# kfkq/DQMC

Measured on AMD Instinct MI355X. Metric: MC sweeps/sec, 2D Hubbard N=256 Ltau=200, higher is better.
Workload: dtype f64; 1 GPU; cfg3: 16x16 Hubbard U=8.0 beta=8.0 Ltau=200 n_stab=10 t=1 mu=-0.1; chains_per_gpu=1, n_chains_total=1, parallelism=independent chains, 1 gpu x 1 chain

## Files before the change

### dqmc_amd/csrc/common.h

```cpp
#pragma once

#include <hip/hip_runtime.h>
#include <cstdint>
#include <memory>
#include <string>

struct dqmc_engine;

namespace dq {

constexpr int WAVE = 64;

void set_error(const std::string& msg);
const char* get_error();

#define DQ_HIP(call)                                                                    \
    do {                                                                                \
        hipError_t _e = (call);                                                         \
        if (_e != hipSuccess) {                                                         \
            ::dq::set_error(std::string(#call) + ": " + hipGetErrorString(_e));         \
            return -2;                                              \
        }                                                                               \
    } while (0)

// ... 22 lines not shown
    double* p = nullptr;
    long stride = 0;
    __host__ __device__ double* at(int c) const { return p + (long)c * stride; }
};
struct CMat {
    const double* p = nullptr;
    long stride = 0;
    CMat() = default;
    __host__ __device__ CMat(const double* p_, long s) : p(p_), stride(s) {}
    __host__ __device__ CMat(const Mat& m) : p(m.p), stride(m.stride) {}
    __host__ __device__ const double* at(int c) const { return p + (long)c * stride; }
};
using Vec = Mat;
using CVec = CMat;

struct GemmDesc {
    CMat A, B;
    Mat C;
    Mat CT{nullptr, 0};
    CVec rs, ks, cs;
    int n = 0;
    int transA = 0;
    int accumulate = 0;
};
int launch_gemm(const GemmDesc& g, int n_chains, hipStream_t s);

int launch_build_expv(const int8_t* fields, long f_stride, int nt, int n, const double* tab_expv ,
                      double* expv, double* invexpv, long v_stride, int n_chains, hipStream_t s);
int launch_split_d(CVec d, Vec dl_inv, Vec ds, double* logsum, int n, int n_chains, hipStream_t s);
int launch_split_d2(CVec d1, Vec dl1, Vec ds1, CVec d2, Vec dl2, Vec ds2, int n, int n_chains, hipStream_t s);
int launch_measure_equal_time(CMat G, double* out, long out_stride, int L1, int L2, int accumulate, int n_chains, hipStream_t s);
int launch_measure_unequal_time(const double* Gtt, const double* Gt0, const double* G0t, double* out, long out_stride, int L1, int L2, int nt,
                                int accumulate, int n_chains, hipStream_t s);
int launch_axpb_identity(CMat in, Mat out, double a, double b, int n, int n_chains, hipStream_t s);
int launch_copy(CMat in, Mat out, long count, int n_chains, hipStream_t s);
int launch_set_identity(Mat out, int n, int n_chains, hipStream_t s);
int launch_transpose_scale(CMat in, Mat out, CVec rs, int n, int n_chains, hipStream_t s);
int launch_max_abs_diff(CMat A, CMat B, double* err, long err_stride, int n, int n_chains, hipStream_t s);
int launch_add_scaled_cols(CMat A, CMat B, CVec cs, Mat C, int n, int n_chains, hipStream_t s);
int launch_scale_rows(CMat in, CVec rs, Mat out, int n, int n_chains, hipStream_t s);
struct DevStats { double acc_rate, max_err, sum_err, n_err; long long n_accepted, n_proposed; };
int launch_fold_stats(DevStats* st, const int* acc, long acc_stride, int n_slices, const double* err, long err_stride, int n_err,
                      int n, int nt, int n_chains, hipStream_t s);

struct QrWork {
    double* tau; long tau_stride;
// ... 11 lines not shown
int launch_qr_panel(Mat A, Mat L, QrWork w, int n, int n_chains, hipStream_t s);
long qrcp_coop_sync_granules(int n);
int qrcp_coop_workgroups(int n, int n_chains);
enum class QrFamily { Panel, ColumnOwner, Cooperative, Streaming };
int launch_to_ldr(QrFamily f, Mat A, Mat L, Vec d, Mat R, QrWork w, int n, int n_chains, hipStream_t s);

int launch_lu_blocked(Mat A, int* perm, long perm_stride, int* rowpos, long rowpos_stride, double* logabsdet, int accumulate_logdet,
                      int* info, int n, int n_chains, hipStream_t s);
int launch_lu_solve(CMat LU, const int* perm, long perm_stride, Mat X, CVec dg, int mode, int n, int n_chains, hipStream_t s);

int launch_tri_solve(CMat R, const int* perm, long perm_stride, Mat X, CVec dg, double* scratch, long scratch_stride, int n, int n_chains, hipStream_t s);

bool gj_fused_fits(int n);
bool gj_fused_default(int n);
int launch_gj_solve(Mat A, Mat B, Mat X, Mat SA, double* tinv, int* perm, long perm_stride, int* rowpos, int* rowpos_alt, long rowpos_stride,
                    double* logabsdet, int accumulate_logdet, int* info, int n, int n_chains, bool fused, hipStream_t s);

struct UpdateTables {
    double rb[4][3];
    double delta[4][3];
    double ev[4];
    double iev[4];
    double pad[32];
};
struct UpdateDesc {
    Mat G;
    int8_t* fields; long f_stride;
    double* expv; double* invexpv; long v_stride;
    const UpdateTables* tabs;
    const int32_t* perm; const uint8_t* kprop; const double* u; long rs_stride;
    double* Upanel; double* Wpanel; long panel_stride;
    double* Cpanel = nullptr;
    int* state; long state_stride;
    double* prep; long prep_stride;
    Mat GT{nullptr, 0};
    int gt_valid = 0;
    void* slice_sync = nullptr;
    unsigned slice_epoch = 0;
    int slice_absent_tile = -1;
    int slice_absent_l = -1;
    int slice_late_tile = -1, slice_late_us = 0;
    int* info = nullptr;
    int* acc_out; long acc_stride;
    int n, nt;
};
constexpr int UPDATE_KD = 32;

struct SliceSync {
    unsigned long long seq; unsigned int error; unsigned int solo_count; unsigned int pad[12];
    unsigned int arrive[496];
};
constexpr size_t SLICE_SYNC_BYTES = 2048;
static_assert(sizeof(SliceSync) == SLICE_SYNC_BYTES, "SliceSync layout");
constexpr unsigned SLICE_EPOCH_LIMIT = 1u << 24;
constexpr unsigned SLICE_SOLO_BIT = 1u << 30, SLICE_FINAL_BIT = 1u << 31;
__host__ __device__ inline unsigned slice_tag(unsigned epoch, unsigned window) { return (epoch << 8) | window; }
enum class SlicePath { PersistentWalk, PersistentSubmatrix, Solo, Pairs, PairsTailSolo };
int launch_update_slice(SlicePath path, const UpdateDesc& d, int l, int acc_slot, int n_chains, hipStream_t s);
int launch_update_slice_sm(const UpdateDesc& d, int l, int acc_slot, int n_chains, hipStream_t s);
int slice_flush_workgroups(int n);
bool slice_reserve(int device, int n, int n_chains);
void slice_release(int device, int n, int n_chains);
int launch_rank1(Mat G, int i, double delta, double* scratch , long scratch_stride, int n, int n_chains, hipStream_t s);

int launch_rng_fill(int32_t* perm, uint8_t* kprop, double* u, int n, int nt, unsigned long long seed, unsigned first_chain, unsigned h,
                    int n_chains, hipStream_t s);

// ... 24 lines not shown
```

### dqmc_amd/csrc/engine.hip

```cpp
#include "common.h"
#include "../../include/dqmc_hip.h"

#include <cmath>
#include <cstdlib>
#include <cstring>
#include <map>
#include <memory>
#include <mutex>
#include <vector>

namespace dq {

static thread_local std::string g_err;
void set_error(const std::string& msg) { g_err = msg; }
const char* get_error() { return g_err.c_str(); }

int init_device_kernels(int device) {
    static std::mutex mu; static bool done[64] = {};
    std::lock_guard<std::mutex> lk(mu);
    if (device < 0 || device >= 64) { set_error("device ordinal out of range"); return -1; }
    if (done[device]) return 0;
    DQ_HIP(hipSetDevice(device));
    DQ_TRY(update_init_device()); DQ_TRY(update_sm_init_device()); DQ_TRY(qr_init_device()); DQ_TRY(qr_colown_init_device());
    done[device] = true;
    return 0;
}

struct Switches { bool qr_panel; int qr_panel_fused, gj_fused; bool qr_streaming, walk_submatrix, lu_classic, slice_multikernel; };
static const Switches& switches() {
    static const Switches sw = [] {
        const char* panel = getenv("DQMC_QR_PANEL");
        const char* fused = getenv("DQMC_QR_PANEL_FUSED");
        const char* gj = getenv("DQMC_GJ_FUSED");
        return Switches{!(panel && atoi(panel) == 0), fused ? (atoi(fused) != 0 ? 1 : 0) : -1, gj ? (atoi(gj) != 0 ? 1 : 0) : -1, getenv("DQMC_QR_STREAMING") != nullptr, getenv("DQMC_WALK_SUBMATRIX") != nullptr,
                        getenv("DQMC_LU_CLASSIC") != nullptr, getenv("DQMC_SLICE_MULTIKERNEL") != nullptr};
    }();
    return sw;
}

constexpr int GJ_MAX_N = 1024, GJ_MAX_CHAINS = 8;
constexpr int TRI_MAX_N = 640;

static QrFamily pick_qr(int n, int chains, bool allow_panel) {
    const Switches& sw = switches();
    if (sw.qr_streaming) return QrFamily::Streaming;
    if (allow_panel && sw.qr_panel && n >= 64 && n <= 1024 && n % 16 == 0 && chains <= 8) return QrFamily::Panel;
    if (n <= 256) return QrFamily::ColumnOwner;
    return qrcp_coop_workgroups(n, chains) <= 200 ? QrFamily::Cooperative : QrFamily::Streaming;
}

struct KernelPlan {
    QrFamily qr;
    enum class Solve { GaussJordan, BlockedLu } solve;
    enum class Rinv { Blocked, PerColumn } rinv;
    static KernelPlan pick(int n, int chains) {
        return KernelPlan{pick_qr(n, chains, true),
                          n <= GJ_MAX_N && chains <= GJ_MAX_CHAINS && !switches().lu_classic ? Solve::GaussJordan : Solve::BlockedLu,
                          n <= TRI_MAX_N ? Rinv::Blocked : Rinv::PerColumn};
// ... 424 lines not shown
        DQ_TRY(launch_to_ldr(pick_qr(n, S, false), cur, all.L, all.d, all.R, w, n, S, s));
        const LdrRef last = stack.at(S - 1), own = ib.f.at(S - 1);
        DQ_TRY(launch_copy(own.L, last.L, nn, 1, s));
        DQ_TRY(launch_copy(own.R, last.R, nn, 1, s));
        DQ_HIP(hipMemcpyAsync(last.d.p, own.d.p, sizeof(double) * n, hipMemcpyDeviceToDevice, s));
        DQ_HIP(hipMemcpyAsync(last.jpvt, own.jpvt, sizeof(int) * n, hipMemcpyDeviceToDevice, s));
        *last.tri = true; last.touch();
        for (int i = S - 2; i >= 0; --i) DQ_TRY(ctx.ldr_mul_ldr(stack.at(i + 1), ib.f.at(i), stack.at(i)));
        stack_valid = true;
        gt_valid = false;
        return ctx.inv_I_plus_ldr(stack.at(0), mG(), logdet.get());
    }
    int wrap_forward(int l) {
        if (cb) {
            DQ_TRY(cb_apply(mG(), Mat{nullptr, 0}, ctx.T(0), false, false, CVec(), CVec(), CVec(), CVec(), C, 4));
            gt_valid = use_gt();
            return cb_apply(ctx.T(0), Mat{GT.get(), nn}, mG(), false, true, CVec(), CVec(), iev(l), ev(l), C, 4);
        }
        DQ_TRY(ctx.gemm(CMat(expK.get(), nn), mG(), ctx.T(0)));
        gt_valid = use_gt();
        return ctx.gemm(ctx.T(0), CMat(invexpK.get(), nn), mG(), ev(l), CVec(), iev(l), 0, 0, use_gt() ? Mat{GT.get(), nn} : Mat{nullptr, 0});
    }
    bool piggyback() const { return C == 1 && !cb && n <= 256 && pg_eye != nullptr; }
    int wrap_forward_piggy(int l, const double* Pprev, double* Pnext) {
        GemmDesc g; g.A = CMat(expK.get(), 0); g.B = CMat(G.get(), (long)(Pprev - G.get())); g.C = Mat{ctx.T(0).p, (long)(Pnext - ctx.T(0).p)};
        g.rs = CVec(pg_ones.get(), (long)((expv.get() + (long)(l - 1) * n) - pg_ones.get())); g.n = n;
        DQ_TRY(launch_gemm(g, 2, s));
        gt_valid = use_gt();
        return ctx.gemm(ctx.T(0), CMat(invexpK.get(), nn), mG(), ev(l), CVec(), iev(l), 0, 0, use_gt() ? Mat{GT.get(), nn} : Mat{nullptr, 0});
    }
    int wrap_backward_piggy(int l, const double* Pprev, double* Pnext) {
        DQ_TRY(ctx.gemm(CMat(invexpK.get(), nn), mG(), ctx.T(0), CVec(), iev(l)));
        gt_valid = use_gt();
        GemmDesc g; g.A = CMat(ctx.T(0).p, (long)(Pprev - ctx.T(0).p)); g.B = CMat(expK.get(), 0); g.C = Mat{G.get(), (long)(Pnext - G.get())};
        g.ks = CVec(expv.get() + (long)l * n, 0); g.n = n;
        if (use_gt()) g.CT = Mat{GT.get(), (long)(ctx.T(1).p - GT.get())};
        return launch_gemm(g, 2, s);
    }
    int wrap_backward(int l) {
        if (cb) {
            DQ_TRY(cb_apply(mG(), Mat{nullptr, 0}, ctx.T(0), true, true, iev(l), ev(l), CVec(), CVec(), C, 4));
            gt_valid = use_gt();
            return cb_apply(ctx.T(0), Mat{GT.get(), nn}, mG(), true, false, CVec(), CVec(), CVec(), CVec(), C, 4);
        }
        DQ_TRY(ctx.gemm(CMat(invexpK.get(), nn), mG(), ctx.T(0), CVec(), iev(l)));
        gt_valid = use_gt();
        return ctx.gemm(ctx.T(0), CMat(expK.get(), nn), mG(), CVec(), ev(l), CVec(), 0, 0, use_gt() ? Mat{GT.get(), nn} : Mat{nullptr, 0});
    }
    bool use_gt() const { return n <= 256 || slice_path == SlicePath::PersistentSubmatrix; }
    UpdateDesc udesc() const {
        UpdateDesc d; d.G = mG(); d.fields = fields.get(); d.f_stride = (long)nt * n; d.expv = expv.get(); d.invexpv = invexpv.get(); d.v_stride = (long)nt * n;
        d.tabs = tabs.get(); d.perm = rs_perm.get(); d.kprop = rs_k.get(); d.u = rs_u.get(); d.rs_stride = (long)nt * n; d.Upanel = Upanel.get(); d.Wpanel = Wpanel.get(); d.Cpanel = Cpanel.get();
        d.panel_stride = (long)UPDATE_KD * n; d.state = state.get(); d.state_stride = 4; d.prep = prep.get(); d.prep_stride = 4L * n; d.slice_sync = is_persistent(slice_path) ? slice_sync.get() : nullptr; d.slice_epoch = slice_epoch; d.slice_absent_tile = slice_absent_tile; d.slice_absent_l = slice_absent_l; d.slice_late_tile = slice_late_tile; d.slice_late_us = slice_late_us; d.GT = Mat{GT.get(), nn}; d.gt_valid = gt_valid ? 1 : 0; d.info = ctx.info(); d.acc_out = acc.get(); d.acc_stride = nt; d.n = n; d.nt = nt;
        return d;
    }
    int local_update(int l) {
        hipEvent_t e0 = nullptr, e1 = nullptr;
        if (profiling) {
            if (ev_used == ev_pairs.size()) { hipEvent_t a, b; DQ_HIP(hipEventCreate(&a)); DQ_HIP(hipEventCreate(&b)); ev_pairs.emplace_back(a, b); }
            e0 = ev_pairs[ev_used].first; e1 = ev_pairs[ev_used].second; ++ev_used;
            DQ_HIP(hipEventRecord(e0, s));
        }
        if (is_persistent(slice_path)) {
            if (++slice_epoch >= SLICE_EPOCH_LIMIT) { DQ_HIP(hipMemsetAsync(slice_sync.get(), 0, (size_t)C * SLICE_SYNC_BYTES, s)); slice_epoch = 1; }
        }
        DQ_TRY(launch_update_slice(slice_path, udesc(), l, l, C, s));
        if (profiling) DQ_HIP(hipEventRecord(e1, s));
        return 0;
    }
    int check_stream(const char* who, const int32_t* perm, const uint8_t* kprop, const double* u, size_t rows) {
        if (!perm || !kprop || !u) { set_error(std::string(who) + ": null random-stream pointer"); return DQMC_EINVAL; }
        seen.assign((size_t)n, 0);
        for (size_t row = 0; row < rows; ++row) {
            const int32_t* pr = perm + row * n; const uint8_t* kr = kprop + row * n; const unsigned char mark = (unsigned char)(1 + (row & 1));
            if ((row & 1) == 0) std::fill(seen.begin(), seen.end(), 0);
            for (int idx = 0; idx < n; ++idx) {
                const int32_t i = pr[idx];
                if (i < 0 || i >= n || seen[i] == mark || kr[idx] > 2) { set_error(std::string(who) + ": perm is not a permutation of the sites, or kprop > 2"); return DQMC_EINVAL; }
                seen[i] = mark;
            }
        }
        return 0;
    }
    int upload_stream(const int32_t* perm, const uint8_t* kprop, const double* u) {
        const size_t cnt = (size_t)C * nt * n;
        DQ_TRY(check_stream("sweep", perm, kprop, u, (size_t)C * nt));
        DQ_HIP(hipEventSynchronize(stage_free));
        char* base = h_stage.get();
        double* hu = reinterpret_cast<double*>(base);
// ... 1 lines not shown
        uint8_t* hk = reinterpret_cast<uint8_t*>(base + cnt * (sizeof(double) + sizeof(int32_t)));
        std::memcpy(hu, u, cnt * sizeof(double)); std::memcpy(hp, perm, cnt * sizeof(int32_t)); std::memcpy(hk, kprop, cnt);
        DQ_HIP(hipMemcpyAsync(rs_u.get(), hu, cnt * sizeof(double), hipMemcpyHostToDevice, s));
        DQ_HIP(hipMemcpyAsync(rs_perm.get(), hp, cnt * sizeof(int32_t), hipMemcpyHostToDevice, s));
        DQ_HIP(hipMemcpyAsync(rs_k.get(), hk, cnt, hipMemcpyHostToDevice, s));
        DQ_HIP(hipEventRecord(stage_free, s));
        return 0;
    }
    int fill_stream(uint32_t h) {
        return launch_rng_fill(rs_perm.get(), rs_k.get(), rs_u.get(), n, nt, rng_seed, rng_first_chain, h, C, s);
    }
    int stage_stream(const char* who, const int32_t* perm, const uint8_t* kprop, const double* u) {
        if (perm && kprop && u) return upload_stream(perm, kprop, u);
        if (perm || kprop || u) { set_error(std::string(who) + ": pass all three random-stream arrays or none"); return DQMC_EINVAL; }
        if (!rng_seeded) { set_error(std::string(who) + ": null random-stream pointer (the engine draws its own stream only after dqmc_rng_seed)"); return DQMC_EINVAL; }
        if (rng_counter == UINT32_MAX) { set_error(std::string(who) + ": the half-sweep counter of this seed is used up (2^32 - 1)"); return DQMC_ERANGE; }
        DQ_TRY(fill_stream(rng_counter));
        ++rng_counter;
        return 0;
    }
    int sweep_fwd() {
        int n_err = 0;
        DQ_HIP(hipMemsetAsync(err.get(), 0, sizeof(double) * C * n_stack, s));
        const bool pg = piggyback();
        double* Pcur = bb0.get(); double* Pnxt = bb1.get();
        for (int l = 0; l < nt; ++l) {
            const int is = stack_idx(l), loc = local_l(l);
            if (pg && loc >= 1) { DQ_TRY(wrap_forward_piggy(l, loc == 1 ? pg_eye.get() : Pcur, Pnxt)); std::swap(Pcur, Pnxt); }
            else DQ_TRY(wrap_forward(l));
            DQ_TRY(local_update(l));
            if (loc == loc_l_end[is]) {
                std::swap(G, Gtmp);
                Mat bb;
                if (pg) {
                    if (loc == 0) DQ_TRY(launch_scale_rows(CMat(expK.get(), nn), ev(l), Mat{Pnxt, nn}, n, C, s));
                    else DQ_TRY(ctx.gemm(CMat(expK.get(), nn), CMat(Pcur, nn), Mat{Pnxt, nn}, ev(l)));
                    std::swap(Pcur, Pnxt); bb = Mat{Pcur, nn};
                } else DQ_TRY(Bbar(is, &bb));
                if (is == 0) DQ_TRY(ctx.to_ldr(bb, stack.at(0)));
                else DQ_TRY(ctx.mat_mul_ldr(bb, stack.at(is - 1), stack.at(is)));
                gt_valid = false;
                if (l == nt - 1) DQ_TRY(ctx.inv_I_plus_ldr(stack.at(is), mG(), logdet.get()));
                else DQ_TRY(ctx.inv_I_plus_ldr_mul_ldr(stack.at(is), stack.at(is + 1), mG()));
                DQ_TRY(launch_max_abs_diff(CMat(Gtmp.get(), nn), mG(), err.get() + n_err, n_stack, n, C, s));
                ++n_err;
            }
        }
        return launch_fold_stats(dstats.get(), acc.get(), nt, nt, err.get(), n_stack, n_err, n, nt, C, s);
    }
    int sweep_bwd() {
        int n_err = 0;
        DQ_HIP(hipMemsetAsync(err.get(), 0, sizeof(double) * C * n_stack, s));
        const bool pg = piggyback();
        double* Pcur = bb0.get(); double* Pnxt = bb1.get();
        for (int l = nt - 1; l >= 0; --l) {
            DQ_TRY(local_update(l));
            const int is = stack_idx(l);
            if (pg) { DQ_TRY(wrap_backward_piggy(l, local_l(l) == loc_l_end[is] ? pg_eye.get() : Pcur, Pnxt)); std::swap(Pcur, Pnxt); }
            else DQ_TRY(wrap_backward(l));
            if (local_l(l) == 0) {
                std::swap(G, Gtmp);
                Mat bb;
                if (pg) bb = Mat{Pcur, nn}; else DQ_TRY(Bbar(is, &bb));
                if (is == n_stack - 1) DQ_TRY(ctx.to_ldr(bb, stack.at(is)));
                else DQ_TRY(ctx.ldr_mul_mat(stack.at(is + 1), bb, stack.at(is)));
                gt_valid = false;
                if (l == 0) DQ_TRY(ctx.inv_I_plus_ldr(stack.at(is), mG(), logdet.get()));
                else {
                    DQ_TRY(ctx.inv_I_plus_ldr_mul_ldr(stack.at(is - 1), stack.at(is), mG(), use_gt() ? Mat{GT.get(), nn} : Mat{nullptr, 0}));
                    gt_valid = use_gt();
                    if (gt_check && gt_valid) {
                        DQ_TRY(launch_transpose_scale(mG(), ctx.T(0), CVec(), n, C, s));
                        DQ_TRY(launch_max_abs_diff(CMat(GT.get(), nn), ctx.T(0), gt_err.get(), 1, n, C, s));
                        ++gt_checks;
                    }
                }
                DQ_TRY(launch_max_abs_diff(CMat(Gtmp.get(), nn), mG(), err.get() + n_err, n_stack, n, C, s));
                ++n_err;
            }
        }
        return launch_fold_stats(dstats.get(), acc.get(), nt, nt, err.get(), n_stack, n_err, n, nt, C, s);
    }
// ... 536 lines not shown
```

### dqmc_amd/csrc/gemm.hip

```cpp
#include "common.h"
#include <cstdlib>

namespace dq {

using d4 = __attribute__((ext_vector_type(4))) double;

template <bool TRANSA, bool GUARD>
__global__ __launch_bounds__(256) void gemm_kernel(GemmDesc g, int tiles_per_dim) {
    const int chain = blockIdx.y;
    const int n = g.n;
    const double* __restrict__ A = g.A.at(chain);
    const double* __restrict__ B = g.B.at(chain);
    double* __restrict__ C = g.C.at(chain);
    const double* __restrict__ ks = g.ks.p ? g.ks.at(chain) : nullptr;

    const int lane = threadIdx.x & 63;
    const int wave = threadIdx.x >> 6;
    const int bt_i = blockIdx.x % tiles_per_dim, bt_j = blockIdx.x / tiles_per_dim;
    const int i0 = bt_i * 32 + (wave & 1) * 16;
    const int j0 = bt_j * 32 + (wave >> 1) * 16;
    if (GUARD && (i0 >= n || j0 >= n)) return;

    const int r = lane & 15, kk = lane >> 4;
    const int ia = i0 + r;
    const int jb = j0 + r;
    const bool ia_ok = !GUARD || ia < n, jb_ok = !GUARD || jb < n;

    d4 acc = {0.0, 0.0, 0.0, 0.0};
// ... 16 lines not shown
#pragma unroll
        for (int s = 0; s < 4; ++s) acc = __builtin_amdgcn_mfma_f64_16x16x4f64(bv[s], av[s], acc, 0, 0, 0);
    }
    if (ia_ok) {
        const double rsv = g.rs.p ? g.rs.at(chain)[ia] : 1.0;
#pragma unroll
        for (int reg = 0; reg < 4; ++reg) {
            const int j = j0 + kk + 4 * reg;
            if (!GUARD || j < n) {
                double v = acc[reg] * rsv;
                if (g.cs.p) v *= g.cs.at(chain)[j];
                double* dst = C + ia + (long)n * j;
                if (g.accumulate) v += *dst;
                *dst = v;
            }
        }
    }
}

template <bool TRANSA, int KQ >
__global__ __launch_bounds__(256) void gemm_splitk_kernel(GemmDesc g, int tiles_per_dim) {
    __shared__ double part[4][4][64];
    const int chain = blockIdx.y;
    const int n = g.n;
    const double* __restrict__ A = g.A.at(chain);
    const double* __restrict__ B = g.B.at(chain);
    double* __restrict__ C = g.C.at(chain);
    const double* __restrict__ ks = g.ks.p ? g.ks.at(chain) : nullptr;
    const int lane = threadIdx.x & 63, wave = threadIdx.x >> 6;
    const int i0 = (blockIdx.x % tiles_per_dim) * 16, j0 = (blockIdx.x / tiles_per_dim) * 16;
    const int r = lane & 15, kk = lane >> 4;
    const int ia = min(i0 + r, n - 1), jb = min(j0 + r, n - 1);
    const bool ia_ok = i0 + r < n, jb_ok = j0 + r < n;
    const int kbeg = wave * KQ;
    constexpr int NB = KQ / 16;
    double av[NB][4], bv[NB][4];
#pragma unroll
    for (int b = 0; b < NB; ++b) {
#pragma unroll
        for (int s = 0; s < 4; ++s) {
            const int k = kbeg + 16 * b + 4 * kk + s;
            const int kc = min(k, n - 1);
            double a = TRANSA ? A[kc + (long)n * ia] : A[ia + (long)n * kc];
            double bb = B[kc + (long)n * jb];
            if (ks) a *= ks[kc];
            const bool ok = k < n;
            av[b][s] = (ok && ia_ok) ? a : 0.0;
            bv[b][s] = (ok && jb_ok) ? bb : 0.0;
        }
    }
    d4 acc = {0.0, 0.0, 0.0, 0.0};
#pragma unroll
    for (int b = 0; b < NB; ++b)
#pragma unroll
        for (int s = 0; s < 4; ++s) acc = __builtin_amdgcn_mfma_f64_16x16x4f64(bv[b][s], av[b][s], acc, 0, 0, 0);
#pragma unroll
    for (int reg = 0; reg < 4; ++reg) part[wave][reg][lane] = acc[reg];
    __syncthreads();
    const double v4 = part[0][wave][lane] + part[1][wave][lane] + part[2][wave][lane] + part[3][wave][lane];
    const int j = j0 + kk + 4 * wave;
    if (ia_ok && j < n) {
        double v = v4;
        if (g.rs.p) v *= g.rs.at(chain)[i0 + r];
        if (g.cs.p) v *= g.cs.at(chain)[j];
        double* dst = C + (i0 + r) + (long)n * j;
        if (g.accumulate) v += *dst;
        *dst = v;
        if (g.CT.p) g.CT.at(chain)[j + (long)n * (i0 + r)] = v;
    }
}

template <bool TRANSA>
__global__ __launch_bounds__(256) void gemm_tile64_kernel(GemmDesc g, int tiles_per_dim) {
    constexpr int LDT = 80;
    __shared__ double As[2][16][LDT];
    __shared__ double Bs[2][16][LDT];
    const int tiles2 = tiles_per_dim * tiles_per_dim;
    const int total = tiles2 * (int)gridDim.y;
    int lin = (int)blockIdx.x + tiles2 * (int)blockIdx.y;
    if ((total & 7) == 0) lin = (lin & 7) * (total >> 3) + (lin >> 3);
    const int chain = lin / tiles2, tile = lin % tiles2;
    const int n = g.n;
    const double* __restrict__ A = g.A.at(chain);
    const double* __restrict__ B = g.B.at(chain);
    double* __restrict__ C = g.C.at(chain);
    const double* __restrict__ ks = g.ks.p ? g.ks.at(chain) : nullptr;
    const int t = threadIdx.x, lane = t & 63, wave = t >> 6;
    const int i0 = (tile % tiles_per_dim) * 64, j0 = (tile / tiles_per_dim) * 64;
    const int r = lane & 15, kk = lane >> 4;
    const int wi = (wave & 1) * 32, wj = (wave >> 1) * 32;
    const int ai = t & 63, akq = t >> 6;
    const int bkp = t & 7, bj = t >> 3;
// ... 159 lines not shown
                    else acc = __builtin_amdgcn_mfma_f64_16x16x4f64(Bs[(wj + r) * PK + k], av, acc, 0, 0, 0);
                }
            }
        }
    }
#pragma unroll
    for (int u = 0; u < D; ++u)
#pragma unroll
        for (int s = 0; s < NL; ++s) asm volatile("s_waitcnt vmcnt(0)" : "+v"(qa[u][s]), "+v"(qb[u][s]), "+v"(qk[u][s]) :: "memory");
    const int i = i0 + wi + r;
    const double rsv = (g.rs.p && i < n) ? g.rs.at(chain)[i] : 1.0;
#pragma unroll
    for (int reg = 0; reg < 4; ++reg) {
        const int jl = wj + kk + 4 * reg, j = j0 + jl;
        double v = (acc[reg] + acc2[reg]) * rsv;
        if (i < n && j < n) {
            if (g.cs.p) v *= g.cs.at(chain)[j];
            double* dst = C + i + (long)n * j;
            if (g.accumulate) v += *dst;
            *dst = v;
        }
        Ct[wi + r][jl] = v;
    }
    if (g.CT.p) {
        __syncthreads();
        double* __restrict__ CT = g.CT.at(chain);
#pragma unroll
        for (int s = 0; s < 4; ++s) {
            const int il = rhi + 8 * s;
            if (i0 + il < n && j0 + rlo < n) CT[(j0 + rlo) + (long)n * (i0 + il)] = Ct[il][rlo];
        }
    }
}

template <int KQ>
static void launch_splitk(const GemmDesc& g, int n_chains, hipStream_t s) {
    const int tiles = (g.n + 15) / 16;
    dim3 grid(tiles * tiles, n_chains), block(256);
    if (g.transA) hipLaunchKernelGGL((gemm_splitk_kernel<true, KQ>), grid, block, 0, s, g, tiles);
    else hipLaunchKernelGGL((gemm_splitk_kernel<false, KQ>), grid, block, 0, s, g, tiles);
}

static int launch_gemm_main(const GemmDesc& g, int n_chains, hipStream_t s, bool* ct_done);

int launch_gemm(const GemmDesc& g, int n_chains, hipStream_t s) {
    bool ct_done = false;
    if (int rc = launch_gemm_main(g, n_chains, s, &ct_done)) return rc;
    if (g.CT.p && !ct_done) return launch_transpose_scale(CMat(g.C.p, g.C.stride), g.CT, CVec(), g.n, n_chains, s);
    return 0;
}

static int launch_gemm_main(const GemmDesc& g, int n_chains, hipStream_t s, bool* ct_done) {
    const int n = g.n;
    if (n % 64 == 0 && (long)n_chains * (n / 64) * (n / 64) >= 256) {
        const int tiles = n / 64;
        dim3 grid(tiles * tiles, n_chains), block(256);
        if (g.transA) hipLaunchKernelGGL((gemm_tile64_kernel<true>), grid, block, 0, s, g, tiles);
        else hipLaunchKernelGGL((gemm_tile64_kernel<false>), grid, block, 0, s, g, tiles);
        DQ_HIP(hipGetLastError());
        return 0;
    }
    if (n >= 384) {
        const int T = (n + 31) / 32, chunk = (T * T + 7) / 8;
        dim3 grid(8 * chunk, n_chains), block(256);
#define DQ_ST(TA, KSC) hipLaunchKernelGGL((gemm_stage32_kernel<TA, KSC, 32>), grid, block, 0, s, g, T, chunk)
        if (g.transA) { if (g.ks.p) DQ_ST(true, true); else DQ_ST(true, false); } else { if (g.ks.p) DQ_ST(false, true); else DQ_ST(false, false); }
#undef DQ_ST
        DQ_HIP(hipGetLastError());
        *ct_done = true;
        return 0;
    }
    if (n <= 640) {
        const int kq = ((n + 3) / 4 + 15) / 16 * 16;
        if (kq <= 16) launch_splitk<16>(g, n_chains, s);
        else if (kq <= 32) launch_splitk<32>(g, n_chains, s);
        else if (kq <= 48) launch_splitk<48>(g, n_chains, s);
        else if (kq <= 64) launch_splitk<64>(g, n_chains, s);
        else if (kq <= 96) launch_splitk<96>(g, n_chains, s);
        else if (kq <= 128) launch_splitk<128>(g, n_chains, s);
        else launch_splitk<160>(g, n_chains, s);
        DQ_HIP(hipGetLastError());
        *ct_done = true;
        return 0;
    }
    const int tiles = (n + 31) / 32;
    dim3 grid(tiles * tiles, n_chains), block(256);
    const bool guard = (n % 32) != 0;
    if (g.transA) {
        if (guard) hipLaunchKernelGGL((gemm_kernel<true, true>), grid, block, 0, s, g, tiles);
        else hipLaunchKernelGGL((gemm_kernel<true, false>), grid, block, 0, s, g, tiles);
    } else {
        if (guard) hipLaunchKernelGGL((gemm_kernel<false, true>), grid, block, 0, s, g, tiles);
        else hipLaunchKernelGGL((gemm_kernel<false, false>), grid, block, 0, s, g, tiles);
    }
    DQ_HIP(hipGetLastError());
    return 0;
// ... 4 lines not shown
```

### dqmc_amd/csrc/update.hip

```cpp
#include "common.h"
#include <cstdlib>
#include <mutex>
#include "wave.h"

namespace dq {

using d4 = __attribute__((ext_vector_type(4))) double;

__constant__ int c_proposal[4][3] = {{1, 2, 3}, {0, 2, 3}, {0, 1, 3}, {0, 1, 2}};

constexpr int SCAN_PF = 8;

__device__ __forceinline__ double ld_coh(const double* p) {
    return __longlong_as_double((long long)__hip_atomic_load(reinterpret_cast<const unsigned long long*>(p), __ATOMIC_RELAXED, __HIP_MEMORY_SCOPE_AGENT));
}
__device__ __forceinline__ void st_coh(double* p, double x) {
    __hip_atomic_store(reinterpret_cast<unsigned long long*>(p), (unsigned long long)__double_as_longlong(x), __ATOMIC_RELAXED, __HIP_MEMORY_SCOPE_AGENT);
}

__host__ __device__ inline size_t scan_lds_bytes(int n, int kd, bool regs) {
    const size_t base = (((size_t)16 * kd * n + (size_t)n * 32 + 256 + (size_t)n * 4 + (size_t)n) + 63) & ~(size_t)63;
    return base + (regs ? (size_t)n * 8 + 4 * (UPDATE_KD + 4) : 0);
}

__device__ __forceinline__ void lds_barrier() {
    asm volatile("s_waitcnt lgkmcnt(0)" ::: "memory");
// ... 516 lines not shown
            if (4 * s >= k) break;
            const int m = 4 * s + kk;
            const bool ok = m < k;
            const int mc = min(m, k - 1);
            const double um = (ok && a_ok) ? UW[mc * n + a].x : 0.0, wm = (ok && b_ok) ? UW[mc * n + b].y : 0.0;
            acc = __builtin_amdgcn_mfma_f64_16x16x4f64(wm, um, acc, 0, 0, 0);
            acc_t = __builtin_amdgcn_mfma_f64_16x16x4f64(um, wm, acc_t, 0, 0, 0);
        }
#pragma unroll
        for (int reg = 0; reg < 4; ++reg) {
            const int bb = b0 + kk + 4 * reg, aa = a0 + kk + 4 * reg;
            if (a_ok && bb < n) G[a + (long)n * bb] = gv[q][reg] + acc[reg];
            if (b_ok && aa < n) GT[b + (long)n * aa] = gt[q][reg] + acc_t[reg];
        }
    }
}

__device__ __attribute__((noinline)) void solo_flush(double* G, double* GT, const double2* UW, int n, int k) {
    const int lane = threadIdx.x & 63, wave = threadIdx.x >> 6;
    const int tiles16 = (n + 15) / 16, n_st = tiles16 * tiles16;
    for (int st = wave; st < n_st; st += 4 * 4) flush_tiles_lds<4>(G, GT, UW, st, 4, n_st, tiles16, n, k, lane);
}

template <int NFIX, int KFIX>
__global__ __launch_bounds__(256) DQ_WALK_REGS void slice_kernel(UpdateDesc d, SliceSync* sync_p, int l, int acc_slot, int kd_arg, int tiles_arg, int* info) {
    extern __shared__ __attribute__((aligned(16))) unsigned char smem[];
    const int chain = blockIdx.y;
    const int n = NFIX ? NFIX : d.n;
    const int kd = KFIX ? KFIX : kd_arg;
    const int tiles_per_dim = NFIX ? (NFIX + 31) / 32 : tiles_arg;
    const int F = tiles_per_dim * tiles_per_dim;
    SliceSync* sy = sync_p + chain;
    double* __restrict__ G = d.G.at(chain);
    double* __restrict__ GT = d.GT.at(chain);
    double* __restrict__ Up = d.Upanel + (long)chain * d.panel_stride;
    double* __restrict__ Wp = d.Wpanel + (long)chain * d.panel_stride;
    const int t = threadIdx.x, lane = t & 63, wave = t >> 6;
    const unsigned epoch = d.slice_epoch;

    if (blockIdx.x > 0) {
        const int tile = blockIdx.x - 1;
        if (tile == d.slice_absent_tile && (d.slice_absent_l < 0 || d.slice_absent_l == l)) return;
        if (tile == d.slice_late_tile) {
            const unsigned long long t0 = wall_clock64();
            while (wall_clock64() - t0 < 100ull * (unsigned long long)d.slice_late_us) __builtin_amdgcn_s_sleep(64);
        }
        const int a0 = (tile % tiles_per_dim) * 32 + (wave & 1) * 16;
        const int b0 = (tile / tiles_per_dim) * 32 + (wave >> 1) * 16;
        if (t == 0) __hip_atomic_store(&sy->arrive[tile], slice_tag(epoch, 0), __ATOMIC_RELAXED, __HIP_MEMORY_SCOPE_AGENT);
        unsigned long long* bcast = reinterpret_cast<unsigned long long*>(smem);
        for (unsigned win = 1;; ++win) {
            if (wave == 0) {
                unsigned long long word = 0; unsigned spins = 0; bool give_up = false;
                for (;;) {
                    word = __hip_atomic_load(&sy->seq, __ATOMIC_RELAXED, __HIP_MEMORY_SCOPE_AGENT);
                    const unsigned tag = (unsigned)(word >> 32);
                    if (tag == slice_tag(epoch, win)) break;
                    if ((tag >> 8) == (slice_tag(epoch, 0) >> 8)) {
                        if ((unsigned)word & SLICE_SOLO_BIT) break;
                        if ((tag & 0xffu) > win) { give_up = true; break; }
                    }
                    if (++spins > SLICE_SPIN_LIMIT) { give_up = true; break; }
// ... 167 lines not shown
    return true;
}
void slice_release(int device, int n, int n_chains) {
    if (device < 0 || device >= 64) return;
    std::lock_guard<std::mutex> lk(g_resv_mu);
    g_resv_used[device] -= slice_workgroups(n, n_chains);
}

int update_init_device() {
    DQ_HIP(hipFuncSetAttribute(reinterpret_cast<const void*>(scan_kernel<256>), hipFuncAttributeMaxDynamicSharedMemorySize, 160 * 1024));
    DQ_HIP(hipFuncSetAttribute(reinterpret_cast<const void*>(scan_kernel<1024>), hipFuncAttributeMaxDynamicSharedMemorySize, 160 * 1024));
    DQ_HIP(hipFuncSetAttribute(reinterpret_cast<const void*>(slice_kernel<0, 0>), hipFuncAttributeMaxDynamicSharedMemorySize, 160 * 1024));
    DQ_HIP(hipFuncSetAttribute(reinterpret_cast<const void*>(slice_kernel<256, UPDATE_KD>), hipFuncAttributeMaxDynamicSharedMemorySize, 160 * 1024));
    DQ_HIP(hipFuncSetAttribute(reinterpret_cast<const void*>(slice_solo_kernel), hipFuncAttributeMaxDynamicSharedMemorySize, 160 * 1024));
    return 0;
}

int launch_update_slice(SlicePath path, const UpdateDesc& d, int l, int acc_slot, int n_chains, hipStream_t s) {
    const int n = d.n;
    if (n > 1024) { set_error("local update kernel supports n_sites <= 1024"); return -1; }
    const int kd = pick_kd(n);
    const int threads = ((n + 63) / 64) * 64;
    const bool regs = threads <= 256;
    const size_t lds = scan_lds_bytes(n, kd, regs);
    const int tiles = (n + 31) / 32;
    if (!regs && path != SlicePath::Pairs && path != SlicePath::PersistentSubmatrix) { set_error("local update: the walk kernels of update.hip need n_sites <= 256"); return -1; }
    if (regs || path == SlicePath::PersistentSubmatrix) {
        if (!d.GT.p) { set_error("local update: transposed workspace missing"); return -1; }
        if (!d.gt_valid) { if (int rc = launch_transpose_scale(CMat(d.G.p, d.G.stride), d.GT, CVec(), n, n_chains, s)) return rc; }
    }
    switch (path) {
    case SlicePath::PersistentSubmatrix: return launch_update_slice_sm(d, l, acc_slot, n_chains, s);
    case SlicePath::PersistentWalk:
        if (!d.slice_sync) { set_error("persistent slice kernel: hand-off words missing"); return -1; }
        if (n == 256 && kd == UPDATE_KD)
            hipLaunchKernelGGL((slice_kernel<256, UPDATE_KD>), dim3(1 + tiles * tiles, n_chains), dim3(256), lds, s, d, reinterpret_cast<SliceSync*>(d.slice_sync), l, acc_slot, kd,
                               tiles, d.info);
        else
            hipLaunchKernelGGL((slice_kernel<0, 0>), dim3(1 + tiles * tiles, n_chains), dim3(256), lds, s, d, reinterpret_cast<SliceSync*>(d.slice_sync), l, acc_slot, kd,
                               tiles, d.info);
        DQ_HIP(hipGetLastError());
        return 0;
    case SlicePath::Solo:
        hipLaunchKernelGGL(slice_solo_kernel, dim3(1, n_chains), dim3(256), lds, s, d, l, acc_slot, kd, 0);
        DQ_HIP(hipGetLastError());
        return 0;
    case SlicePath::Pairs: case SlicePath::PairsTailSolo: break;
    }
    int windows = (n + kd - 1) / kd;
    const bool tail_solo = path == SlicePath::PairsTailSolo && windows > 4;
    if (tail_solo) windows = 4;
    for (int w = 0; w < windows; ++w) {
        if (regs) {
            hipLaunchKernelGGL(scan_kernel<256>, dim3(1, n_chains), dim3(threads), lds, s, d, l, acc_slot, w == 0 ? 1 : 0, kd);
            hipLaunchKernelGGL(flush_kernel<true>, dim3(tiles * tiles, n_chains), dim3(256), 0, s, d, tiles, kd);
        } else {
            hipLaunchKernelGGL(scan_kernel<1024>, dim3(1, n_chains), dim3(threads), lds, s, d, l, acc_slot, w == 0 ? 1 : 0, kd);
            hipLaunchKernelGGL(flush_kernel<false>, dim3(tiles * tiles, n_chains), dim3(256), 0, s, d, tiles, kd);
        }
    }
    if (tail_solo) {
        hipLaunchKernelGGL(slice_solo_kernel, dim3(1, n_chains), dim3(256), lds, s, d, l, acc_slot, kd, 1);
// ... 36 lines not shown
```

Measured before the change: 13.21 sweeps/s.

## Fuse the stabilization B-product GEMM into the persistent walk kernel as extra workgroups

The running product of B matrices was computed by a separate two-chain split-K GEMM launch piggybacked on the wrap. It now runs on extra workgroups appended to the persistent local-update slice kernel, each computing a 2x2 block of 16x16 split-K tiles. This overlaps the product with the sequential Metropolis walk and removes a launch per slice. The wrap GEMM then covers only G, and the backward sweep needs an extra GEMM at block ends. The trade-off is more workgroups and LDS pressure competing with the walk kernel, which relies on persistent workgroups.

```diff
diff --git a/dqmc_amd/csrc/common.h b/dqmc_amd/csrc/common.h
--- a/dqmc_amd/csrc/common.h
+++ b/dqmc_amd/csrc/common.h
@@ -68,6 +68,7 @@
     int n = 0;
     int transA = 0;
     int accumulate = 0;
+    int ct_chains = 1 << 30;
 };
 int launch_gemm(const GemmDesc& g, int n_chains, hipStream_t s);
 
@@ -125,6 +126,14 @@
     double ev[4];
     double iev[4];
     double pad[32];
+};
+struct BbarDesc {
+    const double* A = nullptr;
+    const double* B = nullptr;
+    double* C = nullptr;
+    const double* scale = nullptr;
+    int scale_k = 0;
+    int n = 0;
 };
 struct UpdateDesc {
     Mat G;
@@ -146,6 +155,7 @@
     int* info = nullptr;
     int* acc_out; long acc_stride;
     int n, nt;
+    BbarDesc bbar;
 };
 constexpr int UPDATE_KD = 32;
 
diff --git a/dqmc_amd/csrc/engine.hip b/dqmc_amd/csrc/engine.hip
--- a/dqmc_amd/csrc/engine.hip
+++ b/dqmc_amd/csrc/engine.hip
@@ -26,14 +26,15 @@
     return 0;
 }
 
-struct Switches { bool qr_panel; int qr_panel_fused, gj_fused; bool qr_streaming, walk_submatrix, lu_classic, slice_multikernel; };
+struct Switches { bool qr_panel; int qr_panel_fused, gj_fused; bool qr_streaming, walk_submatrix, lu_classic, slice_multikernel; int bbar_rider; };
 static const Switches& switches() {
     static const Switches sw = [] {
         const char* panel = getenv("DQMC_QR_PANEL");
         const char* fused = getenv("DQMC_QR_PANEL_FUSED");
         const char* gj = getenv("DQMC_GJ_FUSED");
+        const char* rider = getenv("DQMC_BBAR_RIDER");
         return Switches{!(panel && atoi(panel) == 0), fused ? (atoi(fused) != 0 ? 1 : 0) : -1, gj ? (atoi(gj) != 0 ? 1 : 0) : -1, getenv("DQMC_QR_STREAMING") != nullptr, getenv("DQMC_WALK_SUBMATRIX") != nullptr,
-                        getenv("DQMC_LU_CLASSIC") != nullptr, getenv("DQMC_SLICE_MULTIKERNEL") != nullptr};
+                        getenv("DQMC_LU_CLASSIC") != nullptr, getenv("DQMC_SLICE_MULTIKERNEL") != nullptr, rider ? (atoi(rider) != 0 ? 1 : 0) : -1};
     }();
     return sw;
 }
@@ -504,6 +505,13 @@
         return ctx.gemm(ctx.T(0), CMat(invexpK.get(), nn), mG(), ev(l), CVec(), iev(l), 0, 0, use_gt() ? Mat{GT.get(), nn} : Mat{nullptr, 0});
     }
     bool piggyback() const { return C == 1 && !cb && n <= 256 && pg_eye != nullptr; }
+    bool bbar_rides() const {
+        const int sw = switches().bbar_rider, t = (n + 15) / 16;
+        return piggyback() && slice_path == SlicePath::PersistentWalk && (sw < 0 ? 2 * t * t > 256 : sw == 1);
+    }
+    static BbarDesc rider(const double* A, const double* B, double* Cout, const double* scale, bool scale_k, int n) {
+        BbarDesc b; b.A = A; b.B = B; b.C = Cout; b.scale = scale; b.scale_k = scale_k ? 1 : 0; b.n = n; return b;
+    }
     int wrap_forward_piggy(int l, const double* Pprev, double* Pnext) {
         GemmDesc g; g.A = CMat(expK.get(), 0); g.B = CMat(G.get(), (long)(Pprev - G.get())); g.C = Mat{ctx.T(0).p, (long)(Pnext - ctx.T(0).p)};
         g.rs = CVec(pg_ones.get(), (long)((expv.get() + (long)(l - 1) * n) - pg_ones.get())); g.n = n;
@@ -516,7 +524,7 @@
         gt_valid = use_gt();
         GemmDesc g; g.A = CMat(ctx.T(0).p, (long)(Pprev - ctx.T(0).p)); g.B = CMat(expK.get(), 0); g.C = Mat{G.get(), (long)(Pnext - G.get())};
         g.ks = CVec(expv.get() + (long)l * n, 0); g.n = n;
-        if (use_gt()) g.CT = Mat{GT.get(), (long)(ctx.T(1).p - GT.get())};
+        if (use_gt()) { g.CT = Mat{GT.get(), 0}; g.ct_chains = 1; }
         return launch_gemm(g, 2, s);
     }
     int wrap_backward(int l) {
@@ -530,13 +538,14 @@
         return ctx.gemm(ctx.T(0), CMat(expK.get(), nn), mG(), CVec(), ev(l), CVec(), 0, 0, use_gt() ? Mat{GT.get(), nn} : Mat{nullptr, 0});
     }
     bool use_gt() const { return n <= 256 || slice_path == SlicePath::PersistentSubmatrix; }
-    UpdateDesc udesc() const {
+    UpdateDesc udesc(const BbarDesc* ride = nullptr) const {
         UpdateDesc d; d.G = mG(); d.fields = fields.get(); d.f_stride = (long)nt * n; d.expv = expv.get(); d.invexpv = invexpv.get(); d.v_stride = (long)nt * n;
         d.tabs = tabs.get(); d.perm = rs_perm.get(); d.kprop = rs_k.get(); d.u = rs_u.get(); d.rs_stride = (long)nt * n; d.Upanel = Upanel.get(); d.Wpanel = Wpanel.get(); d.Cpanel = Cpanel.get();
         d.panel_stride = (long)UPDATE_KD * n; d.state = state.get(); d.state_stride = 4; d.prep = prep.get(); d.prep_stride = 4L * n; d.slice_sync = is_persistent(slice_path) ? slice_sync.get() : nullptr; d.slice_epoch = slice_epoch; d.slice_absent_tile = slice_absent_tile; d.slice_absent_l = slice_absent_l; d.slice_late_tile = slice_late_tile; d.slice_late_us = slice_late_us; d.GT = Mat{GT.get(), nn}; d.gt_valid = gt_valid ? 1 : 0; d.info = ctx.info(); d.acc_out = acc.get(); d.acc_stride = nt; d.n = n; d.nt = nt;
+        if (ride) d.bbar = *ride;
         return d;
     }
-    int local_update(int l) {
+    int local_update(int l, const BbarDesc* ride = nullptr) {
         hipEvent_t e0 = nullptr, e1 = nullptr;
         if (profiling) {
             if (ev_used == ev_pairs.size()) { hipEvent_t a, b; DQ_HIP(hipEventCreate(&a)); DQ_HIP(hipEventCreate(&b)); ev_pairs.emplace_back(a, b); }
@@ -546,7 +555,7 @@
         if (is_persistent(slice_path)) {
             if (++slice_epoch >= SLICE_EPOCH_LIMIT) { DQ_HIP(hipMemsetAsync(slice_sync.get(), 0, (size_t)C * SLICE_SYNC_BYTES, s)); slice_epoch = 1; }
         }
-        DQ_TRY(launch_update_slice(slice_path, udesc(), l, l, C, s));
+        DQ_TRY(launch_update_slice(slice_path, udesc(ride), l, l, C, s));
         if (profiling) DQ_HIP(hipEventRecord(e1, s));
         return 0;
     }
@@ -594,13 +603,19 @@
     int sweep_fwd() {
         int n_err = 0;
         DQ_HIP(hipMemsetAsync(err.get(), 0, sizeof(double) * C * n_stack, s));
-        const bool pg = piggyback();
+        const bool pg = piggyback(), rides = bbar_rides();
         double* Pcur = bb0.get(); double* Pnxt = bb1.get();
         for (int l = 0; l < nt; ++l) {
             const int is = stack_idx(l), loc = local_l(l);
-            if (pg && loc >= 1) { DQ_TRY(wrap_forward_piggy(l, loc == 1 ? pg_eye.get() : Pcur, Pnxt)); std::swap(Pcur, Pnxt); }
-            else DQ_TRY(wrap_forward(l));
-            DQ_TRY(local_update(l));
+            if (pg && loc >= 1 && rides) {
+                DQ_TRY(wrap_forward(l));
+                const BbarDesc b = rider(expK.get(), loc == 1 ? pg_eye.get() : Pcur, Pnxt, expv.get() + (long)(l - 1) * n, false, n);
+                DQ_TRY(local_update(l, &b)); std::swap(Pcur, Pnxt);
+            } else {
+                if (pg && loc >= 1) { DQ_TRY(wrap_forward_piggy(l, loc == 1 ? pg_eye.get() : Pcur, Pnxt)); std::swap(Pcur, Pnxt); }
+                else DQ_TRY(wrap_forward(l));
+                DQ_TRY(local_update(l));
+            }
             if (loc == loc_l_end[is]) {
                 std::swap(G, Gtmp);
                 Mat bb;
@@ -623,13 +638,25 @@
     int sweep_bwd() {
         int n_err = 0;
         DQ_HIP(hipMemsetAsync(err.get(), 0, sizeof(double) * C * n_stack, s));
-        const bool pg = piggyback();
+        const bool pg = piggyback(), rides = bbar_rides();
         double* Pcur = bb0.get(); double* Pnxt = bb1.get();
         for (int l = nt - 1; l >= 0; --l) {
-            DQ_TRY(local_update(l));
             const int is = stack_idx(l);
-            if (pg) { DQ_TRY(wrap_backward_piggy(l, local_l(l) == loc_l_end[is] ? pg_eye.get() : Pcur, Pnxt)); std::swap(Pcur, Pnxt); }
-            else DQ_TRY(wrap_backward(l));
+            if (rides) {
+                if (local_l(l) != loc_l_end[is]) {
+                    const BbarDesc b = rider(local_l(l + 1) == loc_l_end[is] ? pg_eye.get() : Pcur, expK.get(), Pnxt, expv.get() + (long)(l + 1) * n, true, n);
+                    DQ_TRY(local_update(l, &b)); std::swap(Pcur, Pnxt);
+                } else DQ_TRY(local_update(l));
+                DQ_TRY(wrap_backward(l));
+                if (local_l(l) == 0) {
+                    DQ_TRY(ctx.gemm(CMat(loc_l_end[is] == 0 ? pg_eye.get() : Pcur, nn), CMat(expK.get(), nn), Mat{Pnxt, nn}, CVec(), ev(l)));
+                    std::swap(Pcur, Pnxt);
+                }
+            } else {
+                DQ_TRY(local_update(l));
+                if (pg) { DQ_TRY(wrap_backward_piggy(l, local_l(l) == loc_l_end[is] ? pg_eye.get() : Pcur, Pnxt)); std::swap(Pcur, Pnxt); }
+                else DQ_TRY(wrap_backward(l));
+            }
             if (local_l(l) == 0) {
                 std::swap(G, Gtmp);
                 Mat bb;
diff --git a/dqmc_amd/csrc/gemm.hip b/dqmc_amd/csrc/gemm.hip
--- a/dqmc_amd/csrc/gemm.hip
+++ b/dqmc_amd/csrc/gemm.hip
@@ -1,9 +1,8 @@
 #include "common.h"
+#include "gemm_tile.h"
 #include <cstdlib>
 
 namespace dq {
-
-using d4 = __attribute__((ext_vector_type(4))) double;
 
 template <bool TRANSA, bool GUARD>
 __global__ __launch_bounds__(256) void gemm_kernel(GemmDesc g, int tiles_per_dim) {
@@ -66,52 +65,9 @@
 __global__ __launch_bounds__(256) void gemm_splitk_kernel(GemmDesc g, int tiles_per_dim) {
     __shared__ double part[4][4][64];
     const int chain = blockIdx.y;
-    const int n = g.n;
-    const double* __restrict__ A = g.A.at(chain);
-    const double* __restrict__ B = g.B.at(chain);
-    double* __restrict__ C = g.C.at(chain);
-    const double* __restrict__ ks = g.ks.p ? g.ks.at(chain) : nullptr;
-    const int lane = threadIdx.x & 63, wave = threadIdx.x >> 6;
-    const int i0 = (blockIdx.x % tiles_per_dim) * 16, j0 = (blockIdx.x / tiles_per_dim) * 16;
-    const int r = lane & 15, kk = lane >> 4;
-    const int ia = min(i0 + r, n - 1), jb = min(j0 + r, n - 1);
-    const bool ia_ok = i0 + r < n, jb_ok = j0 + r < n;
-    const int kbeg = wave * KQ;
-    constexpr int NB = KQ / 16;
-    double av[NB][4], bv[NB][4];
-#pragma unroll
-    for (int b = 0; b < NB; ++b) {
-#pragma unroll
-        for (int s = 0; s < 4; ++s) {
-            const int k = kbeg + 16 * b + 4 * kk + s;
-            const int kc = min(k, n - 1);
-            double a = TRANSA ? A[kc + (long)n * ia] : A[ia + (long)n * kc];
-            double bb = B[kc + (long)n * jb];
-            if (ks) a *= ks[kc];
-            const bool ok = k < n;
-            av[b][s] = (ok && ia_ok) ? a : 0.0;
-            bv[b][s] = (ok && jb_ok) ? bb : 0.0;
-        }
-    }
-    d4 acc = {0.0, 0.0, 0.0, 0.0};
-#pragma unroll
-    for (int b = 0; b < NB; ++b)
-#pragma unroll
-        for (int s = 0; s < 4; ++s) acc = __builtin_amdgcn_mfma_f64_16x16x4f64(bv[b][s], av[b][s], acc, 0, 0, 0);
-#pragma unroll
-    for (int reg = 0; reg < 4; ++reg) part[wave][reg][lane] = acc[reg];
-    __syncthreads();
-    const double v4 = part[0][wave][lane] + part[1][wave][lane] + part[2][wave][lane] + part[3][wave][lane];
-    const int j = j0 + kk + 4 * wave;
-    if (ia_ok && j < n) {
-        double v = v4;
-        if (g.rs.p) v *= g.rs.at(chain)[i0 + r];
-        if (g.cs.p) v *= g.cs.at(chain)[j];
-        double* dst = C + (i0 + r) + (long)n * j;
-        if (g.accumulate) v += *dst;
-        *dst = v;
-        if (g.CT.p) g.CT.at(chain)[j + (long)n * (i0 + r)] = v;
-    }
+    const SplitkOperands op{g.A.at(chain), g.B.at(chain), g.C.at(chain), g.CT.p && chain < g.ct_chains ? g.CT.at(chain) : nullptr,
+                            g.rs.p ? g.rs.at(chain) : nullptr, g.ks.p ? g.ks.at(chain) : nullptr, g.cs.p ? g.cs.at(chain) : nullptr, g.n, g.accumulate};
+    gemm_splitk_tile<TRANSA, KQ>(op, blockIdx.x, tiles_per_dim, part);
 }
 
 template <bool TRANSA>
@@ -317,7 +273,7 @@
         }
         Ct[wi + r][jl] = v;
     }
-    if (g.CT.p) {
+    if (g.CT.p && chain < g.ct_chains) {
         __syncthreads();
         double* __restrict__ CT = g.CT.at(chain);
 #pragma unroll
@@ -341,7 +297,7 @@
 int launch_gemm(const GemmDesc& g, int n_chains, hipStream_t s) {
     bool ct_done = false;
     if (int rc = launch_gemm_main(g, n_chains, s, &ct_done)) return rc;
-    if (g.CT.p && !ct_done) return launch_transpose_scale(CMat(g.C.p, g.C.stride), g.CT, CVec(), g.n, n_chains, s);
+    if (g.CT.p && !ct_done) return launch_transpose_scale(CMat(g.C.p, g.C.stride), g.CT, CVec(), g.n, n_chains < g.ct_chains ? n_chains : g.ct_chains, s);
     return 0;
 }
 
@@ -366,7 +322,7 @@
         return 0;
     }
     if (n <= 640) {
-        const int kq = ((n + 3) / 4 + 15) / 16 * 16;
+        const int kq = splitk_kq(n);
         if (kq <= 16) launch_splitk<16>(g, n_chains, s);
         else if (kq <= 32) launch_splitk<32>(g, n_chains, s);
         else if (kq <= 48) launch_splitk<48>(g, n_chains, s);
diff --git a/dqmc_amd/csrc/gemm_tile.h b/dqmc_amd/csrc/gemm_tile.h
--- /dev/null
+++ b/dqmc_amd/csrc/gemm_tile.h
@@ -0,0 +1,66 @@
+#pragma once
+#include "common.h"
+
+namespace dq {
+
+using d4 = __attribute__((ext_vector_type(4))) double;
+
+__host__ __device__ inline int splitk_kq(int n) { return ((n + 3) / 4 + 15) / 16 * 16; }
+
+struct SplitkOperands {
+    const double* A; const double* B; double* C; double* CT;
+    const double* rs; const double* ks; const double* cs;
+    int n, accumulate;
+};
+
+template <bool TRANSA, int KQ >
+__device__ __forceinline__ void gemm_splitk_tile(const SplitkOperands& g, int tile, int tiles_per_dim, double (*part)[4][64] ) {
+    const int n = g.n;
+    const double* __restrict__ A = g.A;
+    const double* __restrict__ B = g.B;
+    double* __restrict__ C = g.C;
+    const double* __restrict__ ks = g.ks;
+    const int lane = threadIdx.x & 63, wave = threadIdx.x >> 6;
+    const int i0 = (tile % tiles_per_dim) * 16, j0 = (tile / tiles_per_dim) * 16;
+    const int r = lane & 15, kk = lane >> 4;
+    const int ia = min(i0 + r, n - 1), jb = min(j0 + r, n - 1);
+    const bool ia_ok = i0 + r < n, jb_ok = j0 + r < n;
+    const int kbeg = wave * KQ;
+    constexpr int NB = KQ / 16;
+    double av[NB][4], bv[NB][4];
+#pragma unroll
+    for (int b = 0; b < NB; ++b) {
+#pragma unroll
+        for (int s = 0; s < 4; ++s) {
+            const int k = kbeg + 16 * b + 4 * kk + s;
+            const int kc = min(k, n - 1);
+            double a = TRANSA ? A[kc + (long)n * ia] : A[ia + (long)n * kc];
+            double bb = B[kc + (long)n * jb];
+            if (ks) a *= ks[kc];
+            const bool ok = k < n;
+            av[b][s] = (ok && ia_ok) ? a : 0.0;
+            bv[b][s] = (ok && jb_ok) ? bb : 0.0;
+        }
+    }
+    d4 acc = {0.0, 0.0, 0.0, 0.0};
+#pragma unroll
+    for (int b = 0; b < NB; ++b)
+#pragma unroll
+        for (int s = 0; s < 4; ++s) acc = __builtin_amdgcn_mfma_f64_16x16x4f64(bv[b][s], av[b][s], acc, 0, 0, 0);
+#pragma unroll
+    for (int reg = 0; reg < 4; ++reg) part[wave][reg][lane] = acc[reg];
+    __syncthreads();
+    const double v4 = part[0][wave][lane] + part[1][wave][lane] + part[2][wave][lane] + part[3][wave][lane];
+    const int j = j0 + kk + 4 * wave;
+    if (ia_ok && j < n) {
+        double v = v4;
+        if (g.rs) v *= g.rs[i0 + r];
+        if (g.cs) v *= g.cs[j];
+        double* dst = C + (i0 + r) + (long)n * j;
+        if (g.accumulate) v += *dst;
+        *dst = v;
+        if (g.CT) g.CT[j + (long)n * (i0 + r)] = v;
+    }
+}
+
+}
diff --git a/dqmc_amd/csrc/update.hip b/dqmc_amd/csrc/update.hip
--- a/dqmc_amd/csrc/update.hip
+++ b/dqmc_amd/csrc/update.hip
@@ -2,6 +2,7 @@
 #include <cstdlib>
 #include <mutex>
 #include "wave.h"
+#include "gemm_tile.h"
 
 namespace dq {
 
@@ -564,6 +565,33 @@
     for (int st = wave; st < n_st; st += 4 * 4) flush_tiles_lds<4>(G, GT, UW, st, 4, n_st, tiles16, n, k, lane);
 }
 
+#define DQ_AS_GLOBAL __attribute__((address_space(1)))
+#define DQ_AS_LDS __attribute__((address_space(3)))
+constexpr int BBAR_SIDE = 2;
+__device__ __attribute__((noinline)) void bbar_tile(DQ_AS_GLOBAL const double* A, DQ_AS_GLOBAL const double* B, DQ_AS_GLOBAL double* C, DQ_AS_GLOBAL const double* scale_g,
+                                                     int scale_k, int n, int tile, DQ_AS_LDS double* lds) {
+    double (*part)[4][64] = reinterpret_cast<double (*)[4][64]>((double*)lds);
+    const double* scale = (const double*)scale_g;
+    const SplitkOperands op{(const double*)A, (const double*)B, (double*)C, nullptr, scale_k ? nullptr : scale, scale_k ? scale : nullptr, nullptr, n, 0};
+    const int tiles16 = (n + 15) / 16, kq = splitk_kq(n);
+    if (kq <= 16) gemm_splitk_tile<false, 16>(op, tile, tiles16, part);
+    else if (kq <= 32) gemm_splitk_tile<false, 32>(op, tile, tiles16, part);
+    else if (kq <= 48) gemm_splitk_tile<false, 48>(op, tile, tiles16, part);
+    else gemm_splitk_tile<false, 64>(op, tile, tiles16, part);
+}
+__device__ __forceinline__ void bbar_role(const BbarDesc& b, int n, int wg, unsigned char* smem) {
+    const int tiles16 = (n + 15) / 16, blocks = (tiles16 + BBAR_SIDE - 1) / BBAR_SIDE;
+    for (int q = 0; q < BBAR_SIDE * BBAR_SIDE; ++q) {
+        const int ti = BBAR_SIDE * (wg % blocks) + q % BBAR_SIDE, tj = BBAR_SIDE * (wg / blocks) + q / BBAR_SIDE;
+        if (ti >= tiles16 || tj >= tiles16) continue;
+        if (q) __syncthreads();
+        bbar_tile((DQ_AS_GLOBAL const double*)b.A, (DQ_AS_GLOBAL const double*)b.B, (DQ_AS_GLOBAL double*)b.C, (DQ_AS_GLOBAL const double*)b.scale, b.scale_k, n,
+                  ti + tiles16 * tj, (DQ_AS_LDS double*)smem);
+    }
+}
+static int bbar_role_workgroups(int n) { const int blocks = ((n + 15) / 16 + BBAR_SIDE - 1) / BBAR_SIDE; return blocks * blocks; }
+constexpr size_t BBAR_LDS_BYTES = 4 * 4 * 64 * sizeof(double);
+
 template <int NFIX, int KFIX>
 __global__ __launch_bounds__(256) DQ_WALK_REGS void slice_kernel(UpdateDesc d, SliceSync* sync_p, int l, int acc_slot, int kd_arg, int tiles_arg, int* info) {
     extern __shared__ __attribute__((aligned(16))) unsigned char smem[];
@@ -580,6 +608,10 @@
     const int t = threadIdx.x, lane = t & 63, wave = t >> 6;
     const unsigned epoch = d.slice_epoch;
 
+    if ((int)blockIdx.x > F) {
+        bbar_role(d.bbar, n, (int)blockIdx.x - 1 - F, smem);
+        return;
+    }
     if (blockIdx.x > 0) {
         const int tile = blockIdx.x - 1;
         if (tile == d.slice_absent_tile && (d.slice_absent_l < 0 || d.slice_absent_l == l)) return;
@@ -793,8 +825,14 @@
     const int kd = pick_kd(n);
     const int threads = ((n + 63) / 64) * 64;
     const bool regs = threads <= 256;
-    const size_t lds = scan_lds_bytes(n, kd, regs);
+    size_t lds = scan_lds_bytes(n, kd, regs);
     const int tiles = (n + 31) / 32;
+    int rider_wgs = 0;
+    if (d.bbar.A) {
+        if (path != SlicePath::PersistentWalk || n_chains != 1 || d.bbar.n != n || !d.bbar.B || !d.bbar.C) { set_error("local update: a product rides on the persistent walk kernel of one chain only"); return -1; }
+        rider_wgs = bbar_role_workgroups(n);
+        if (lds < BBAR_LDS_BYTES) lds = BBAR_LDS_BYTES;
+    }
     if (!regs && path != SlicePath::Pairs && path != SlicePath::PersistentSubmatrix) { set_error("local update: the walk kernels of update.hip need n_sites <= 256"); return -1; }
     if (regs || path == SlicePath::PersistentSubmatrix) {
         if (!d.GT.p) { set_error("local update: transposed workspace missing"); return -1; }
@@ -805,10 +843,10 @@
     case SlicePath::PersistentWalk:
         if (!d.slice_sync) { set_error("persistent slice kernel: hand-off words missing"); return -1; }
         if (n == 256 && kd == UPDATE_KD)
-            hipLaunchKernelGGL((slice_kernel<256, UPDATE_KD>), dim3(1 + tiles * tiles, n_chains), dim3(256), lds, s, d, reinterpret_cast<SliceSync*>(d.slice_sync), l, acc_slot, kd,
+            hipLaunchKernelGGL((slice_kernel<256, UPDATE_KD>), dim3(1 + tiles * tiles + rider_wgs, n_chains), dim3(256), lds, s, d, reinterpret_cast<SliceSync*>(d.slice_sync), l, acc_slot, kd,
                                tiles, d.info);
         else
-            hipLaunchKernelGGL((slice_kernel<0, 0>), dim3(1 + tiles * tiles, n_chains), dim3(256), lds, s, d, reinterpret_cast<SliceSync*>(d.slice_sync), l, acc_slot, kd,
+            hipLaunchKernelGGL((slice_kernel<0, 0>), dim3(1 + tiles * tiles + rider_wgs, n_chains), dim3(256), lds, s, d, reinterpret_cast<SliceSync*>(d.slice_sync), l, acc_slot, kd,
                                tiles, d.info);
         DQ_HIP(hipGetLastError());
         return 0;
```

Result: no change. 13.28 sweeps/s (median of 6 runs) (+0.6%).
